# thu-nics/MixDQ

Hardware: AMD Instinct MI355X
Metric: sdxl_turbo_unet_w8a8_images_per_sec (higher is better)
Workload: dtype int8; 1 GPU; sdxl_turbo_unet_w8a8_1024px_bs1_1step; global_batch=1, per_gpu_batch=1, px=1024, latent=128, unet_forwards_per_image=1, unet_rows_per_image=1, graphs_cached=1, w_config=weight/uniform_8, a_config=act/act_8.00, bos=True, parallelism=dp1 (batch-sharded replicas, no step-loop collective), hip_graph=True, producer_fusions=True, swap_glue=False, w4_kernel_layers=0, quantizable_layers=794

## Files before the change

mixdq_amd/csrc/iconv.hip:

```cpp
#include <type_traits>

#include "iconv.h"

namespace mixdq {
namespace {

__device__ uint4 g_zero_page;

__device__ __forceinline__ void dma16(const void* gsrc, char* lds_wave_base) {
  __builtin_amdgcn_global_load_lds((const __attribute__((address_space(1))) void*)gsrc,
                                   (__attribute__((address_space(3))) void*)lds_wave_base, 16, 0, 0);
}

__device__ __forceinline__ uint32_t add_f16x2_(uint32_t a, uint32_t b) {
  const v2h ah = *reinterpret_cast<const v2h*>(&a), bh = *reinterpret_cast<const v2h*>(&b);
  v2f r = __builtin_convertvector(ah, v2f) + __builtin_convertvector(bh, v2f);
  asm("" : "+v"(r));
  const v2h h = __builtin_convertvector(r, v2h);
  return *reinterpret_cast<const uint32_t*>(&h);
}

template <int TH, int TW, int BN, int CK, int WNG = 1, bool W4 = false>
struct HaloGeom {
  static constexpr int BM = TH * TW;
  static constexpr int HWP = TW + 2, HP = (TH + 2) * HWP;
  static constexpr int KSPLIT = CK / 64;
  static constexpr int NWAVES = 8, NTHREADS = 512, WPX = NWAVES / KSPLIT / WNG;
  static constexpr int PPP = 1024 / CK, LPP = CK / 16;
  static constexpr int H_NI = ((HP + PPP - 1) / PPP + NWAVES - 1) / NWAVES;
  static constexpr int HALO_BYTES = H_NI * NWAVES * 1024;
  static constexpr int WROW = W4 ? CK / 2 : CK, WLPP = WROW / 16;
  static constexpr int W_TAP = BN * WROW;
  static constexpr int W_PIECES = (3 * W_TAP + 1023) / 1024;
  static constexpr int W_STAGE = W_PIECES * 1024;
  static constexpr int W_LO = W_PIECES / NWAVES, W_REM = W_PIECES % NWAVES, W_NI = W_LO + (W_REM ? 1 : 0);
  static constexpr int HALO_OFF = 3 * W_STAGE;
  static constexpr int MAIN_BYTES = HALO_OFF + 2 * HALO_BYTES;
  static constexpr int CS_STRIDE = BN * 2 + 16;
  static constexpr int WTN = BN / WNG;
  static constexpr int WTM = BM / WPX, TM = WTM / 16, TN = WTN / 16;
  static constexpr int PART_BYTES = (KSPLIT - 1) * WPX * TM * TN * 4 * 64 * 4;
  static constexpr int SMEM = MAIN_BYTES + 9 * BN * 4 + BN * 6;
  static_assert(CK == 64 || CK == 128, "one or two 64-byte MFMA k-steps per chunk");
  static_assert((W4 || W_TAP % 1024 == 0) && W_TAP % 256 == 0 && WTN % 16 == 0 && WTM % 16 == 0,
                "whole DMA pieces (int8) / LDS bank rows / MFMA tiles");
  static_assert(WNG == 1 || KSPLIT == 1, "channel wave groups only without the k-split");
  static_assert(BM * CS_STRIDE + PART_BYTES <= MAIN_BYTES, "epilogue staging overlays the main buffers");
  static_assert(SMEM <= 160 * 1024, "LDS is 160 KiB per CU");
  static_assert(H_NI + 2 * W_NI <= 63, "vmcnt is a 6-bit counter");
  __device__ static int swz(int row) {
    if (CK == 64) return ((row >> 2) & 1) << 1;
    return TW == 16 ? ((row >> 1) & 3) << 1 : (row >> 1) & 7;
  }
  __device__ static int wswz(int row) { return WROW == 64 ? (row >> 2) & 3 : (row >> 3) & 1; }
};

template <int TH, int TW, int BN, int CK, int WNG = 1, bool W4 = false>
__global__ __launch_bounds__(512, 2) void conv3x3_halo_kernel(const HaloConvArgs p) {
  using G = HaloGeom<TH, TW, BN, CK, WNG, W4>;
  constexpr int BM = G::BM, HWP = G::HWP, HP = G::HP, TM = G::TM, TN = G::TN;
  constexpr int CS_STRIDE = G::CS_STRIDE;
  MIXDQ_ARGS_NOW(p.X, p.Wt, p.scale, p.bias, p.table, p.zp, p.D, p.res, p.res_div, p.NI, p.H, p.W, p.C,
                 p.K, p.unfused, p.ups);
  const float zpv = *(const __attribute__((address_space(4))) float*)p.zp;
  extern __shared__ __attribute__((aligned(16))) char smem[];
  const int tid = threadIdx.x, lane = tid & 63;
  const int wid = __builtin_amdgcn_readfirstlane(tid >> 6);
  const int kg = WNG == 1 ? wid / G::WPX : 0;
  const int wn = WNG == 1 ? 0 : wid / G::WPX;
  const int wm = wid % G::WPX;
  const int lrow = lane & 15, lkq = lane >> 4;

  const int tiles_x = p.W / TW, tiles_y = p.H / TH, tiles_n = (p.K + BN - 1) / BN;
  const int tiles_m = p.NI * tiles_y * tiles_x;
  const int nwg = tiles_m * tiles_n;
  const int bid = blockIdx.x;
  const int xcd = bid % kNumXCD, q8 = nwg / kNumXCD, r8 = nwg % kNumXCD;
  const int wg = (xcd < r8 ? xcd * (q8 + 1) : r8 * (q8 + 1) + (xcd - r8) * q8) + bid / kNumXCD;
  constexpr int GM = 8;
  const int per_group = GM * tiles_n;
  const int group = wg / per_group;
  const int first_m = group * GM;
  const int gsz = min(GM, tiles_m - first_m);
  const int rem = wg - group * per_group;
  const int tile_n = rem / gsz, tile_m = first_m + (rem - tile_n * gsz);
  const int img = tile_m / (tiles_y * tiles_x);
  const int trem = tile_m - img * (tiles_y * tiles_x);
  const int y0 = (trem / tiles_x) * TH, x0 = (trem % tiles_x) * TW;
  const int n0 = tile_n * BN;
  const int C = p.C;
  const int nch = (C + CK - 1) / CK;
  const char* zero = reinterpret_cast<const char*>(&g_zero_page);
  const int sh = p.ups ? 1 : 0, SW = p.W >> sh;
  const int8_t* ximg = p.X + (int64_t)img * (p.H >> sh) * SW * C;

  const bool has_bias = p.bias != nullptr;
  v4f pre_tab, pre_sc;
  uint2 pre_bs;
  const bool tab_on = tid < 9 * (BN / 4), pre_on = tid < BN / 4;
  const int tab_q = tid % (BN / 4), tab_c = tid / (BN / 4);
  const bool tab_in = n0 + tab_q * 4 < p.K;
  if (tab_on) {
    const int rc = tab_c / 3, cc = tab_c % 3;
    const int rlo = rc == 1 ? 1 : 0, rhi = rc == 2 ? 1 : 2, slo = cc == 1 ? 1 : 0, shi = cc == 2 ? 1 : 2;
    const int cls = ((rlo * 3 + rhi) * 3 + slo) * 3 + shi;
    const int n = tab_in ? n0 + tab_q * 4 : 0;
    pre_tab = *reinterpret_cast<const v4f*>(p.table + (int64_t)cls * p.K + n);
    if (pre_on) {
      pre_sc = *reinterpret_cast<const v4f*>(p.scale + n);
      if (has_bias) pre_bs = *reinterpret_cast<const uint2*>(p.bias + n);
    }
  }

  uint32_t h_off[G::H_NI];
  int h_c16[G::H_NI];
  bool h_ok[G::H_NI];
#pragma unroll
  for (int j = 0; j < G::H_NI; ++j) {
    const int h = (wid + 8 * j) * G::PPP + lane / G::LPP;
    const int hy = h / HWP, hx = h - hy * HWP;
    const int iy = y0 - 1 + hy, ix = x0 - 1 + hx;
    const int c16 = ((lane % G::LPP) ^ G::swz(h)) << 4;
    h_ok[j] = h < HP && (unsigned)iy < (unsigned)p.H && (unsigned)ix < (unsigned)p.W;
    h_off[j] = h_ok[j] ? (uint32_t)((iy >> sh) * SW + (ix >> sh)) * (uint32_t)C + c16 : 0u;
    h_c16[j] = c16;
  }
  uint32_t w_off[G::W_NI];
  int w_c16[G::W_NI];
  bool w_ok[G::W_NI];
#pragma unroll
  for (int j = 0; j < G::W_NI; ++j) {
    const int q = wid + 8 * j;
    if constexpr (W4) {
      const int L = q * 64 + lane;
      const int s = L / (BN * G::WLPP), rem = L - s * (BN * G::WLPP);
      const int row = rem / G::WLPP;
      const int c16 = ((rem % G::WLPP) ^ G::wswz(row)) << 4;
      w_ok[j] = L < 3 * BN * G::WLPP && n0 + row < p.K;
      w_off[j] = w_ok[j] ? (uint32_t)(n0 + row) * (uint32_t)(9 * (C >> 1)) + (uint32_t)(s * (C >> 1)) + c16 : 0u;
      w_c16[j] = c16;
    } else {
      const int s = q / (BN / G::PPP), row = (q - s * (BN / G::PPP)) * G::PPP + lane / G::LPP;
      const int c16 = ((lane % G::LPP) ^ G::swz(row)) << 4;
      w_ok[j] = q < G::W_PIECES && n0 + row < p.K;
      w_off[j] = w_ok[j] ? (uint32_t)(n0 + row) * (uint32_t)(9 * C) + (uint32_t)(s * C) + c16 : 0u;
      w_c16[j] = c16;
    }
  }
  auto stage_halo = [&](int chunk, int buf) {
    char* dst = smem + G::HALO_OFF + buf * G::HALO_BYTES;
    const int c0 = chunk * CK;
    const bool live = chunk < nch;
#pragma unroll
    for (int j = 0; j < G::H_NI; ++j) {
      const bool ok = live && h_ok[j] && c0 + h_c16[j] < C;
      dma16(ok ? (const void*)(ximg + h_off[j] + c0) : (const void*)zero, dst + (wid + 8 * j) * 1024);
    }
  };
  auto stage_w = [&](int chunk, int r) {
    char* dst = smem + r * G::W_STAGE;
    const int c0 = W4 ? chunk * (CK / 2) : chunk * CK;
    const int cend = W4 ? C >> 1 : C;
    const bool live = chunk < nch;
    const int8_t* base = p.Wt + (r * 3) * cend + c0;
#pragma unroll
    for (int j = 0; j < G::W_NI; ++j) {
      if (j >= G::W_LO && wid >= G::W_REM) continue;
      const bool ok = live && w_ok[j] && c0 + w_c16[j] < cend;
      dma16(ok ? (const void*)(base + w_off[j]) : (const void*)zero, dst + (wid + 8 * j) * 1024);
    }
  };
  auto wait_row = [&](auto r_c) {
    constexpr int r = decltype(r_c)::value;
    constexpr int extra = r == 1 ? G::H_NI : 0;
    if constexpr (G::W_REM == 0) {
      asm volatile("s_waitcnt vmcnt(%0)\n\ts_barrier" ::"n"(G::W_LO + extra) : "memory");
    } else {
      if (wid < G::W_REM) asm volatile("s_waitcnt vmcnt(%0)\n\ts_barrier" ::"n"(G::W_NI + extra) : "memory");
      else asm volatile("s_waitcnt vmcnt(%0)\n\ts_barrier" ::"n"(G::W_LO + extra) : "memory");
    }
  };

  int x_rd[TM][9];
#pragma unroll
  for (int t = 0; t < TM; ++t) {
    const int i = wm * G::WTM + t * 16 + lrow;
    const int hb = (i / TW) * HWP + (i % TW);
#pragma unroll
    for (int tap = 0; tap < 9; ++tap) {
      const int h = hb + (tap / 3) * HWP + (tap % 3);
      x_rd[t][tap] = G::HALO_OFF + h * CK + (((kg * 4 + lkq) ^ G::swz(h)) << 4);
    }
  }
  int w_rd[TN];
#pragma unroll
  for (int tn = 0; tn < TN; ++tn) {
    const int row = wn * G::WTN + tn * 16 + lrow;
    if constexpr (W4)
      w_rd[tn] = row * G::WROW + (((kg * 2 + (lkq >> 1)) ^ G::wswz(row)) << 4) + (lkq & 1) * 8;
    else
      w_rd[tn] = row * CK + (((kg * 4 + lkq) ^ G::swz(row)) << 4);
  }
  v4i acc[TN][TM];
#pragma unroll
  for (int a = 0; a < TN; ++a)
#pragma unroll
    for (int b = 0; b < TM; ++b) acc[a][b] = v4i{0, 0, 0, 0};

  stage_halo(0, 0);
  stage_w(0, 0);
  stage_w(0, 1);
  auto chunk_body = [&](auto hb_c, int ch) {
    constexpr int HB = decltype(hb_c)::value;
#pragma unroll
    for (int r = 0; r < 3; ++r) {
      if (r == 0) wait_row(std::integral_constant<int, 0>{});
      else if (r == 1) wait_row(std::integral_constant<int, 1>{});
      else wait_row(std::integral_constant<int, 2>{});
      if (r == 0) stage_halo(ch + 1, HB ^ 1);
      stage_w(ch + (r + 2) / 3, (r + 2) % 3);
      const char* Ws = smem + r * G::W_STAGE;
      const char* Hs = smem + HB * G::HALO_BYTES;
#pragma unroll
      for (int s = 0; s < 3; ++s) {
        v4i wf[TN], xf[TM];
#pragma unroll
        for (int t = 0; t < TM; ++t) xf[t] = *reinterpret_cast<const v4i*>(Hs + x_rd[t][r * 3 + s]);
#pragma unroll
        for (int tn = 0; tn < TN; ++tn) {
          if constexpr (W4) {
            const uint2 w = *reinterpret_cast<const uint2*>(Ws + s * G::W_TAP + w_rd[tn]);
            wf[tn] = v4i{(int)(w.x & 0xF0F0F0F0u), (int)((w.x << 4) & 0xF0F0F0F0u),
                         (int)(w.y & 0xF0F0F0F0u), (int)((w.y << 4) & 0xF0F0F0F0u)};
          } else {
            wf[tn] = *reinterpret_cast<const v4i*>(Ws + s * G::W_TAP + w_rd[tn]);
          }
        }
#pragma unroll
        for (int tn = 0; tn < TN; ++tn)
#pragma unroll
          for (int t = 0; t < TM; ++t)
            acc[tn][t] = __builtin_amdgcn_mfma_i32_16x16x64_i8(wf[tn], xf[t], acc[tn][t], 0, 0, 0);
      }
    }
  };
  for (int ch = 0; ch < nch; ch += 2) {
    chunk_body(std::integral_constant<int, 0>{}, ch);
    if (ch + 1 < nch) chunk_body(std::integral_constant<int, 1>{}, ch + 1);
  }
  asm volatile("s_waitcnt vmcnt(0)" ::: "memory");

  constexpr int PARAM_OFF = G::MAIN_BYTES;
  float* P_TAB = reinterpret_cast<float*>(smem + PARAM_OFF);
  float* P_SC = P_TAB + 9 * BN;
  __half* P_BS = reinterpret_cast<__half*>(P_SC + BN);
  if (tab_on) {
    const v4f zero4 = {0.f, 0.f, 0.f, 0.f};
    if constexpr (W4) {
      pre_tab = pre_tab * 16.0f;
      if (pre_on) pre_sc = pre_sc * 0.0625f;
    }
    *reinterpret_cast<v4f*>(P_TAB + tab_c * BN + tab_q * 4) = tab_in ? pre_tab : zero4;
    if (pre_on) {
      *reinterpret_cast<v4f*>(P_SC + tab_q * 4) = tab_in ? pre_sc : zero4;
      *reinterpret_cast<uint2*>(P_BS + tab_q * 4) = tab_in && has_bias ? pre_bs : make_uint2(0u, 0u);
    }
  }
  __syncthreads();
  if constexpr (G::KSPLIT == 2) {
    constexpr int WREGS = TN * TM * 4;
    int* part = reinterpret_cast<int*>(smem + BM * CS_STRIDE) + (wm * WREGS * 64 + lane);
    if (kg != 0) {
#pragma unroll
      for (int a = 0; a < TN; ++a)
#pragma unroll
        for (int b = 0; b < TM; ++b)
#pragma unroll
          for (int e = 0; e < 4; ++e) part[((a * TM + b) * 4 + e) * 64] = acc[a][b][e];
    }
    __syncthreads();
    if (kg == 0) {
#pragma unroll
      for (int a = 0; a < TN; ++a)
#pragma unroll
        for (int b = 0; b < TM; ++b)
#pragma unroll
          for (int e = 0; e < 4; ++e) acc[a][b][e] += part[((a * TM + b) * 4 + e) * 64];
    }
  }
  char* Cs = smem;
  auto to_tile = [&](auto mode_c) {
    constexpr int MODE = decltype(mode_c)::value;
#pragma unroll
    for (int t = 0; t < TM; ++t) {
      const int ml = wm * G::WTM + t * 16 + lrow;
      const int pp = y0 + ml / TW, qq = x0 + ml % TW;
      const int rc = pp == 0 ? 1 : (pp == p.H - 1 ? 2 : 0), cc = qq == 0 ? 1 : (qq == p.W - 1 ? 2 : 0);
      const float* b0row = P_TAB + (rc * 3 + cc) * BN;
#pragma unroll
      for (int tn = 0; tn < TN; ++tn) {
        const int nl = wn * G::WTN + tn * 16 + 4 * lkq;
        v4f b0 = *reinterpret_cast<const v4f*>(b0row + nl);
        b0 = b0 * zpv;
        const v4f sc = *reinterpret_cast<const v4f*>(P_SC + nl);
        v4f bs = {0.f, 0.f, 0.f, 0.f};
        if constexpr (MODE != 0)
          bs = __builtin_convertvector(*reinterpret_cast<const v4h*>(P_BS + nl), v4f);
        uint32_t packed[2];
#pragma unroll
        for (int e2 = 0; e2 < 2; ++e2) {
          v2f x = {(float)acc[tn][t][2 * e2], (float)acc[tn][t][2 * e2 + 1]};
          const v2f b0e = {b0[2 * e2], b0[2 * e2 + 1]};
          const v2f sce = {sc[2 * e2], sc[2 * e2 + 1]};
          const v2f bse = {bs[2 * e2], bs[2 * e2 + 1]};
          v2f r;
          x = x - b0e;
          if constexpr (MODE == 0) r = x * sce;
          else if constexpr (MODE == 2) r = x * sce + bse;
          else r = __builtin_elementwise_fma(x, sce, bse);
          asm("" : "+v"(r));
          const v2h h = __builtin_convertvector(r, v2h);
          packed[e2] = *reinterpret_cast<const uint32_t*>(&h);
        }
        *reinterpret_cast<uint2*>(Cs + ml * CS_STRIDE + nl * 2) = make_uint2(packed[0], packed[1]);
      }
    }
  };
  if (kg == 0) {
    if (!has_bias) to_tile(std::integral_constant<int, 0>{});
    else if (!p.unfused) to_tile(std::integral_constant<int, 1>{});
    else to_tile(std::integral_constant<int, 2>{});
  }
  constexpr int CPRO = BN / 8;
  const bool n8 = (p.K & 7) == 0;
  constexpr int ST_ITERS = (BM * CPRO + G::NTHREADS - 1) / G::NTHREADS;
  static_assert(ST_ITERS <= 10, "residual chunks parked in registers");
  v4i res_late[ST_ITERS];
  const bool res_late_on = p.res != nullptr && n8;
  if (res_late_on) {
#pragma unroll
    for (int it = 0; it < ST_ITERS; ++it) {
      const int idx = min(tid + it * G::NTHREADS, BM * CPRO - 1);
      const int row = idx / CPRO, cc = idx - row * CPRO;
      const int n = n0 + cc * 8 < p.K ? n0 + cc * 8 : 0;
      const int64_t pix = ((int64_t)img * p.H + (y0 + row / TW)) * p.W + (x0 + row % TW);
      res_late[it] = *reinterpret_cast<const v4i*>(p.res + (p.res_div == 1 ? pix : (int64_t)img) * p.K + n);
    }
  }
  __syncthreads();
#pragma unroll
  for (int it = 0; it < ST_ITERS; ++it) {
    const int idx = tid + it * G::NTHREADS;
    if (idx >= BM * CPRO) break;
    const int row = idx / CPRO, cc = idx - row * CPRO;
    const int n = n0 + cc * 8;
    if (n >= p.K) continue;
    const int64_t pix = ((int64_t)img * p.H + (y0 + row / TW)) * p.W + (x0 + row % TW);
    uint4 v = *reinterpret_cast<const uint4*>(Cs + row * CS_STRIDE + cc * 16);
    if (p.res != nullptr) {
      const __half* rp = p.res + (p.res_div == 1 ? pix : (int64_t)img) * p.K + n;
      uint32_t rw[4];
      if (n8) {
        const v4i r = res_late[it];
        rw[0] = (uint32_t)r[0]; rw[1] = (uint32_t)r[1]; rw[2] = (uint32_t)r[2]; rw[3] = (uint32_t)r[3];
      } else {
        const uint2 r0 = *reinterpret_cast<const uint2*>(rp);
        rw[0] = r0.x; rw[1] = r0.y; rw[2] = 0; rw[3] = 0;
        if (n + 8 <= p.K) {
          const uint2 r1 = *reinterpret_cast<const uint2*>(rp + 4);
          rw[2] = r1.x; rw[3] = r1.y;
        }
      }
      uint32_t* vw = reinterpret_cast<uint32_t*>(&v);
#pragma unroll
      for (int e = 0; e < 4; ++e) vw[e] = add_f16x2_(vw[e], rw[e]);
    }
    __half* dst = p.D + pix * p.K + n;
    if (n8) {
      const v4i vv = {(int)v.x, (int)v.y, (int)v.z, (int)v.w};
        __builtin_nontemporal_store(vv, reinterpret_cast<v4i*>(dst));
    } else {
      *reinterpret_cast<uint2*>(dst) = make_uint2(v.x, v.y);
      if (n + 8 <= p.K) *reinterpret_cast<uint2*>(dst + 4) = make_uint2(v.z, v.w);
    }
  }
}

template <int TH, int TW, int BN, int CK, int WNG = 1, bool W4 = false>
int launch_halo(const HaloConvArgs& a, hipStream_t stream) {
  using G = HaloGeom<TH, TW, BN, CK, WNG, W4>;
  static bool seen[64] = {};
  if (const int st = lds_opt_in(reinterpret_cast<const void*>(&conv3x3_halo_kernel<TH, TW, BN, CK, WNG, W4>),
                                G::SMEM, seen))
    return st;
  const int64_t grid = (int64_t)a.NI * (a.H / TH) * (a.W / TW) * ((a.K + BN - 1) / BN);
  if (grid <= 0 || grid > 0x7fffffff) return MIXDQ_ERR_INVALID_ARG;
  conv3x3_halo_kernel<TH, TW, BN, CK, WNG, W4><<<dim3((unsigned)grid), 512, G::SMEM, stream>>>(a);
  return launch_status();
}

}

int halo_conv_select(int NI, int H, int W, int C, int K, int R, int S, int stride, int pad, bool w4) {
  if (R != 3 || S != 3 || stride != 1 || pad != 1 || NI <= 0) return 0;
  if (C % 64 != 0 || K % 4 != 0 || H % 8 != 0 || W % 8 != 0) return 0;
  if ((int64_t)H * W * C >= (1ll << 32) || (int64_t)K * 9 * C >= (1ll << 32)) return 0;
  const int64_t tiles_n = (K + 79) / 80;
  if (H % 16 == 0 && W % 16 == 0 && K % 160 == 0 && (int64_t)NI * (H / 16) * (W / 16) * (K / 160) >= kNumCU)
    return 93;
  if (H % 16 == 0 && W % 16 == 0 && (int64_t)NI * (H / 16) * (W / 16) * tiles_n >= kNumCU) return 92;
  if (w4 && K <= 16) return 0;
  if (W % 16 == 0 && (int64_t)NI * (H / 8) * (W / 16) * tiles_n >= kNumCU) return 90;
  return 91;
}

int halo_conv_launch(const HaloConvArgs& a, int tile, hipStream_t stream, bool w4) {
  if (w4) {
    switch (tile) {
#define X(ID, TH, TW, BN, CK, WNG) case ID: return launch_halo<TH, TW, BN, CK, WNG, true>(a, stream);
      MIXDQ_HALO_TILES(X)
#undef X
      default: return MIXDQ_ERR_INVALID_ARG;
    }
  }
  switch (tile) {
#define X(ID, TH, TW, BN, CK, WNG) case ID: return launch_halo<TH, TW, BN, CK, WNG>(a, stream);
    MIXDQ_HALO_TILES(X)
#undef X
    default: return MIXDQ_ERR_INVALID_ARG;
  }
}

}
```

Before: 92.23 images/s.

## Software-pipeline LDS fragment reads across taps in halo int8 conv kernel

Adds a pipelined main loop for the 3x3 halo convolution that double-buffers MFMA fragments in registers. It issues LDS reads for the next tap (via inline ds_read with immediate offsets) while MFMAs for the current tap run, and uses explicit lgkmcnt waits. Tile 92 also gets a fourth weight stage, and tile 90 staggers DMA issue across wave halves. The first global-to-LDS requests are hoisted ahead of the epilogue parameter loads, and compile-time timestamp probes are added but off by default. The aim is to hide LDS latency and DMA issue behind MFMA work, at the cost of more registers, more LDS for the extra stage, and tighter counter budgets.

```diff
diff --git a/mixdq_amd/csrc/iconv.hip b/mixdq_amd/csrc/iconv.hip
--- a/mixdq_amd/csrc/iconv.hip
+++ b/mixdq_amd/csrc/iconv.hip
@@ -1,11 +1,57 @@
 #include <type_traits>
+#include <utility>
 
 #include "iconv.h"
+
+#ifndef MIXDQ_STAMP
+#define MIXDQ_STAMP 0
+#endif
+#ifndef MIXDQ_HALO_PIPE
+#define MIXDQ_HALO_PIPE -1
+#endif
 
 namespace mixdq {
 namespace {
 
 __device__ uint4 g_zero_page;
+#if MIXDQ_STAMP
+__device__ unsigned long long g_halo_stamps;
+#define MIXDQ_HALO_STAMP(slot)                                                                    \
+  do {                                                                                            \
+    const unsigned long long t_ = __builtin_amdgcn_s_memtime();                                   \
+    const unsigned long long r_ = __builtin_amdgcn_s_memrealtime();                               \
+    const unsigned long long a_ = g_halo_stamps;                                                  \
+    if (a_ != 0 && (threadIdx.x & 63) == 0) {                                                     \
+      auto sp_ = (__attribute__((address_space(1))) unsigned long long*)a_ +                      \
+                 ((size_t)blockIdx.x * 16 + (threadIdx.x >> 6)) * 16;                             \
+      sp_[slot] = t_;                                                                             \
+      if ((slot) == 0) sp_[8] = r_;                                                               \
+      if ((slot) == 7) sp_[9] = r_;                                                               \
+    }                                                                                             \
+  } while (0)
+#else
+#define MIXDQ_HALO_STAMP(slot) do {} while (0)
+#endif
+
+template <class F, int... I>
+__device__ __forceinline__ void static_for_(F&& f, std::integer_sequence<int, I...>) {
+  (f(std::integral_constant<int, I>{}), ...);
+}
+template <int N, class F>
+__device__ __forceinline__ void static_for(F&& f) {
+  static_for_(f, std::make_integer_sequence<int, N>{});
+}
+
+template <int OFF>
+__device__ __forceinline__ void lds_rd128(v4i& d, unsigned addr) {
+  static_assert(OFF >= 0 && OFF < 65536, "ds offset field");
+  asm volatile("ds_read_b128 %0, %1 offset:%2" : "=v"(d) : "v"(addr), "n"(OFF) : "memory");
+}
+template <int OFF>
+__device__ __forceinline__ void lds_rd64(v2i& d, unsigned addr) {
+  static_assert(OFF >= 0 && OFF < 65536, "ds offset field");
+  asm volatile("ds_read_b64 %0, %1 offset:%2" : "=v"(d) : "v"(addr), "n"(OFF) : "memory");
+}
 
 __device__ __forceinline__ void dma16(const void* gsrc, char* lds_wave_base) {
   __builtin_amdgcn_global_load_lds((const __attribute__((address_space(1))) void*)gsrc,
@@ -20,7 +66,7 @@
   return *reinterpret_cast<const uint32_t*>(&h);
 }
 
-template <int TH, int TW, int BN, int CK, int WNG = 1, bool W4 = false>
+template <int TH, int TW, int BN, int CK, int WNG = 1, bool W4 = false, int PIPE = 0>
 struct HaloGeom {
   static constexpr int BM = TH * TW;
   static constexpr int HWP = TW + 2, HP = (TH + 2) * HWP;
@@ -34,7 +80,8 @@
   static constexpr int W_PIECES = (3 * W_TAP + 1023) / 1024;
   static constexpr int W_STAGE = W_PIECES * 1024;
   static constexpr int W_LO = W_PIECES / NWAVES, W_REM = W_PIECES % NWAVES, W_NI = W_LO + (W_REM ? 1 : 0);
-  static constexpr int HALO_OFF = 3 * W_STAGE;
+  static constexpr int WST = PIPE == 2 ? 4 : 3;
+  static constexpr int HALO_OFF = WST * W_STAGE;
   static constexpr int MAIN_BYTES = HALO_OFF + 2 * HALO_BYTES;
   static constexpr int CS_STRIDE = BN * 2 + 16;
   static constexpr int WTN = BN / WNG;
@@ -47,7 +94,8 @@
   static_assert(WNG == 1 || KSPLIT == 1, "channel wave groups only without the k-split");
   static_assert(BM * CS_STRIDE + PART_BYTES <= MAIN_BYTES, "epilogue staging overlays the main buffers");
   static_assert(SMEM <= 160 * 1024, "LDS is 160 KiB per CU");
-  static_assert(H_NI + 2 * W_NI <= 63, "vmcnt is a 6-bit counter");
+  static_assert(H_NI + (WST - 1) * W_NI <= 63, "vmcnt is a 6-bit counter");
+  static_assert(PIPE == 0 || 2 * (TM + TN) <= 15, "lgkmcnt is a 4-bit counter: two taps of fragment reads in flight");
   __device__ static int swz(int row) {
     if (CK == 64) return ((row >> 2) & 1) << 1;
     return TW == 16 ? ((row >> 1) & 3) << 1 : (row >> 1) & 7;
@@ -55,13 +103,14 @@
   __device__ static int wswz(int row) { return WROW == 64 ? (row >> 2) & 3 : (row >> 3) & 1; }
 };
 
-template <int TH, int TW, int BN, int CK, int WNG = 1, bool W4 = false>
+template <int TH, int TW, int BN, int CK, int WNG = 1, bool W4 = false, int PIPE = 0, bool STAG = false>
 __global__ __launch_bounds__(512, 2) void conv3x3_halo_kernel(const HaloConvArgs p) {
-  using G = HaloGeom<TH, TW, BN, CK, WNG, W4>;
-  constexpr int BM = G::BM, HWP = G::HWP, HP = G::HP, TM = G::TM, TN = G::TN;
+  using G = HaloGeom<TH, TW, BN, CK, WNG, W4, PIPE>;
+  constexpr int BM = G::BM, HWP = G::HWP, HP = G::HP, TM = G::TM, TN = G::TN, WST = G::WST;
   constexpr int CS_STRIDE = G::CS_STRIDE;
   MIXDQ_ARGS_NOW(p.X, p.Wt, p.scale, p.bias, p.table, p.zp, p.D, p.res, p.res_div, p.NI, p.H, p.W, p.C,
                  p.K, p.unfused, p.ups);
+  MIXDQ_HALO_STAMP(0);
   const float zpv = *(const __attribute__((address_space(4))) float*)p.zp;
   extern __shared__ __attribute__((aligned(16))) char smem[];
   const int tid = threadIdx.x, lane = tid & 63;
@@ -94,24 +143,6 @@
   const int sh = p.ups ? 1 : 0, SW = p.W >> sh;
   const int8_t* ximg = p.X + (int64_t)img * (p.H >> sh) * SW * C;
 
-  const bool has_bias = p.bias != nullptr;
-  v4f pre_tab, pre_sc;
-  uint2 pre_bs;
-  const bool tab_on = tid < 9 * (BN / 4), pre_on = tid < BN / 4;
-  const int tab_q = tid % (BN / 4), tab_c = tid / (BN / 4);
-  const bool tab_in = n0 + tab_q * 4 < p.K;
-  if (tab_on) {
-    const int rc = tab_c / 3, cc = tab_c % 3;
-    const int rlo = rc == 1 ? 1 : 0, rhi = rc == 2 ? 1 : 2, slo = cc == 1 ? 1 : 0, shi = cc == 2 ? 1 : 2;
-    const int cls = ((rlo * 3 + rhi) * 3 + slo) * 3 + shi;
-    const int n = tab_in ? n0 + tab_q * 4 : 0;
-    pre_tab = *reinterpret_cast<const v4f*>(p.table + (int64_t)cls * p.K + n);
-    if (pre_on) {
-      pre_sc = *reinterpret_cast<const v4f*>(p.scale + n);
-      if (has_bias) pre_bs = *reinterpret_cast<const uint2*>(p.bias + n);
-    }
-  }
-
   uint32_t h_off[G::H_NI];
   int h_c16[G::H_NI];
   bool h_ok[G::H_NI];
@@ -157,8 +188,8 @@
       dma16(ok ? (const void*)(ximg + h_off[j] + c0) : (const void*)zero, dst + (wid + 8 * j) * 1024);
     }
   };
-  auto stage_w = [&](int chunk, int r) {
-    char* dst = smem + r * G::W_STAGE;
+  auto stage_w = [&](int chunk, int r, int stage) {
+    char* dst = smem + stage * G::W_STAGE;
     const int c0 = W4 ? chunk * (CK / 2) : chunk * CK;
     const int cend = W4 ? C >> 1 : C;
     const bool live = chunk < nch;
@@ -181,6 +212,33 @@
     }
   };
 
+  auto first_requests = [&]() {
+    stage_halo(0, 0);
+#pragma unroll
+    for (int r = 0; r < WST - 1; ++r) stage_w(0, r, r);
+    __builtin_amdgcn_sched_barrier(0);
+    MIXDQ_HALO_STAMP(1);
+  };
+  if constexpr (PIPE != 0) first_requests();
+
+  const bool has_bias = p.bias != nullptr;
+  v4f pre_tab, pre_sc;
+  uint2 pre_bs;
+  const bool tab_on = tid < 9 * (BN / 4), pre_on = tid < BN / 4;
+  const int tab_q = tid % (BN / 4), tab_c = tid / (BN / 4);
+  const bool tab_in = n0 + tab_q * 4 < p.K;
+  if (tab_on) {
+    const int rc = tab_c / 3, cc = tab_c % 3;
+    const int rlo = rc == 1 ? 1 : 0, rhi = rc == 2 ? 1 : 2, slo = cc == 1 ? 1 : 0, shi = cc == 2 ? 1 : 2;
+    const int cls = ((rlo * 3 + rhi) * 3 + slo) * 3 + shi;
+    const int n = tab_in ? n0 + tab_q * 4 : 0;
+    pre_tab = *reinterpret_cast<const v4f*>(p.table + (int64_t)cls * p.K + n);
+    if (pre_on) {
+      pre_sc = *reinterpret_cast<const v4f*>(p.scale + n);
+      if (has_bias) pre_bs = *reinterpret_cast<const uint2*>(p.bias + n);
+    }
+  }
+
   int x_rd[TM][9];
 #pragma unroll
   for (int t = 0; t < TM; ++t) {
@@ -206,19 +264,108 @@
   for (int a = 0; a < TN; ++a)
 #pragma unroll
     for (int b = 0; b < TM; ++b) acc[a][b] = v4i{0, 0, 0, 0};
-
-  stage_halo(0, 0);
-  stage_w(0, 0);
-  stage_w(0, 1);
+  if constexpr (PIPE == 0) first_requests();
+
+  [[maybe_unused]] v4i xf2[2][TM];
+  [[maybe_unused]] std::conditional_t<W4, v2i, v4i> wf2[2][TN];
+  const unsigned lds0 = (unsigned)(size_t)(__attribute__((address_space(3))) char*)smem;
+  auto rd_x = [&](auto hb_c, auto tap_c, auto buf_c) {
+    static_for<TM>([&](auto t) {
+      lds_rd128<decltype(hb_c)::value * G::HALO_BYTES>(xf2[decltype(buf_c)::value][decltype(t)::value],
+                                                        lds0 + x_rd[decltype(t)::value][decltype(tap_c)::value]);
+    });
+  };
+  auto rd_w = [&](auto s_c, auto buf_c, unsigned stage_base) {
+    static_for<TN>([&](auto tn) {
+      const unsigned a = lds0 + stage_base + w_rd[decltype(tn)::value];
+      if constexpr (W4) lds_rd64<decltype(s_c)::value * G::W_TAP>(wf2[decltype(buf_c)::value][decltype(tn)::value], a);
+      else lds_rd128<decltype(s_c)::value * G::W_TAP>(wf2[decltype(buf_c)::value][decltype(tn)::value], a);
+    });
+  };
+  auto land = [&](auto n_c, auto buf_c) {
+    asm volatile("s_waitcnt lgkmcnt(%0)" ::"n"(decltype(n_c)::value) : "memory");
+    constexpr int B = decltype(buf_c)::value;
+#pragma unroll
+    for (int t = 0; t < TM; ++t) asm volatile("" : "+v"(xf2[B][t]));
+#pragma unroll
+    for (int tn = 0; tn < TN; ++tn) asm volatile("" : "+v"(wf2[B][tn]));
+    __builtin_amdgcn_sched_barrier(0);
+  };
+  auto mma = [&](auto buf_c) {
+    constexpr int B = decltype(buf_c)::value;
+#pragma unroll
+    for (int tn = 0; tn < TN; ++tn) {
+      v4i w;
+      if constexpr (W4) {
+        const uint32_t lo = (uint32_t)wf2[B][tn][0], hi = (uint32_t)wf2[B][tn][1];
+        w = v4i{(int)(lo & 0xF0F0F0F0u), (int)((lo << 4) & 0xF0F0F0F0u),
+                (int)(hi & 0xF0F0F0F0u), (int)((hi << 4) & 0xF0F0F0F0u)};
+      } else {
+        w = wf2[B][tn];
+      }
+#pragma unroll
+      for (int t = 0; t < TM; ++t)
+        acc[tn][t] = __builtin_amdgcn_mfma_i32_16x16x64_i8(w, xf2[B][t], acc[tn][t], 0, 0, 0);
+    }
+    __builtin_amdgcn_sched_barrier(0);
+  };
+  auto pipe_step = [&](auto hb_c, auto r_c, int ch) {
+    constexpr int HB = decltype(hb_c)::value, R = decltype(r_c)::value;
+    constexpr int P0 = (HB + R) & 1;
+    using B0 = std::integral_constant<int, P0>;
+    using B1 = std::integral_constant<int, P0 ^ 1>;
+    using HBc = std::integral_constant<int, HB>;
+    constexpr int NF = TM + TN;
+    const int g = 3 * ch + R;
+    auto requests = [&]() {
+      if (R == 0) stage_halo(ch + 1, HB ^ 1);
+      if constexpr (WST == 3) stage_w(ch + (R + 2) / 3, (R + 2) % 3, (R + 2) % 3);
+      else stage_w(ch + 1, R, (g + 3) & 3);
+    };
+    const bool late = STAG && wid >= 4;
+    if (!late) requests();
+    const unsigned wbase = (WST == 3 ? R : (g & 3)) * G::W_STAGE;
+    if constexpr (PIPE != 2) rd_w(std::integral_constant<int, 0>{}, B0{}, wbase);
+    rd_x(HBc{}, std::integral_constant<int, R * 3 + 1>{}, B1{});
+    rd_w(std::integral_constant<int, 1>{}, B1{}, wbase);
+    land(std::integral_constant<int, NF>{}, B0{});
+    mma(B0{});
+    if (late) requests();
+    rd_x(HBc{}, std::integral_constant<int, R * 3 + 2>{}, B0{});
+    rd_w(std::integral_constant<int, 2>{}, B0{}, wbase);
+    land(std::integral_constant<int, NF>{}, B1{});
+    mma(B1{});
+    constexpr int NP = PIPE == 2 ? NF : TM;
+    const unsigned wnext = ((g + 1) & 3) * G::W_STAGE;
+    if constexpr (R < 2) rd_x(HBc{}, std::integral_constant<int, (R + 1) * 3>{}, B1{});
+    else rd_x(std::integral_constant<int, HB ^ 1>{}, std::integral_constant<int, 0>{}, B1{});
+    if constexpr (PIPE == 2) rd_w(std::integral_constant<int, 0>{}, B1{}, wnext);
+    land(std::integral_constant<int, NP>{}, B0{});
+    mma(B0{});
+    wait_row(std::integral_constant<int, (R + 1) % 3>{});
+  };
+  auto pipe_first = [&]() {
+    wait_row(std::integral_constant<int, 0>{});
+    MIXDQ_HALO_STAMP(2);
+    rd_x(std::integral_constant<int, 0>{}, std::integral_constant<int, 0>{}, std::integral_constant<int, 0>{});
+    if constexpr (PIPE == 2) rd_w(std::integral_constant<int, 0>{}, std::integral_constant<int, 0>{}, 0u);
+  };
   auto chunk_body = [&](auto hb_c, int ch) {
     constexpr int HB = decltype(hb_c)::value;
+    if constexpr (PIPE != 0) {
+      pipe_step(hb_c, std::integral_constant<int, 0>{}, ch);
+      pipe_step(hb_c, std::integral_constant<int, 1>{}, ch);
+      pipe_step(hb_c, std::integral_constant<int, 2>{}, ch);
+      return;
+    }
 #pragma unroll
     for (int r = 0; r < 3; ++r) {
       if (r == 0) wait_row(std::integral_constant<int, 0>{});
       else if (r == 1) wait_row(std::integral_constant<int, 1>{});
       else wait_row(std::integral_constant<int, 2>{});
+      if (r == 0 && HB == 0 && ch == 0) MIXDQ_HALO_STAMP(2);
       if (r == 0) stage_halo(ch + 1, HB ^ 1);
-      stage_w(ch + (r + 2) / 3, (r + 2) % 3);
+      stage_w(ch + (r + 2) / 3, (r + 2) % 3, (r + 2) % 3);
       const char* Ws = smem + r * G::W_STAGE;
       const char* Hs = smem + HB * G::HALO_BYTES;
 #pragma unroll
@@ -244,11 +391,17 @@
       }
     }
   };
+  if constexpr (PIPE != 0) pipe_first();
   for (int ch = 0; ch < nch; ch += 2) {
     chunk_body(std::integral_constant<int, 0>{}, ch);
     if (ch + 1 < nch) chunk_body(std::integral_constant<int, 1>{}, ch + 1);
   }
   asm volatile("s_waitcnt vmcnt(0)" ::: "memory");
+  if constexpr (PIPE != 0) {
+    land(std::integral_constant<int, 0>{}, std::integral_constant<int, 0>{});
+    land(std::integral_constant<int, 0>{}, std::integral_constant<int, 1>{});
+  }
+  MIXDQ_HALO_STAMP(3);
 
   constexpr int PARAM_OFF = G::MAIN_BYTES;
   float* P_TAB = reinterpret_cast<float*>(smem + PARAM_OFF);
@@ -331,6 +484,7 @@
     else if (!p.unfused) to_tile(std::integral_constant<int, 1>{});
     else to_tile(std::integral_constant<int, 2>{});
   }
+  MIXDQ_HALO_STAMP(5);
   constexpr int CPRO = BN / 8;
   const bool n8 = (p.K & 7) == 0;
   constexpr int ST_ITERS = (BM * CPRO + G::NTHREADS - 1) / G::NTHREADS;
@@ -384,22 +538,56 @@
       if (n + 8 <= p.K) *reinterpret_cast<uint2*>(dst + 4) = make_uint2(v.z, v.w);
     }
   }
-}
-
-template <int TH, int TW, int BN, int CK, int WNG = 1, bool W4 = false>
-int launch_halo(const HaloConvArgs& a, hipStream_t stream) {
-  using G = HaloGeom<TH, TW, BN, CK, WNG, W4>;
+  MIXDQ_HALO_STAMP(7);
+}
+
+constexpr int halo_pipe(int id, bool w4) {
+  if (id == 93) return 0;
+  const bool room4 = !w4 && (id == 92 || id == 91);
+  if (MIXDQ_HALO_PIPE >= 0) return MIXDQ_HALO_PIPE == 2 && !room4 ? 1 : MIXDQ_HALO_PIPE;
+  return !w4 && id == 92 ? 2 : 1;
+}
+
+#ifndef MIXDQ_HALO_STAGGER
+#define MIXDQ_HALO_STAGGER -1
+#endif
+constexpr bool halo_stagger(int id, bool w4) {
+  if (halo_pipe(id, w4) == 0) return false;
+  if (MIXDQ_HALO_STAGGER >= 0) return MIXDQ_HALO_STAGGER != 0;
+  return id == 90;
+}
+
+template <int TH, int TW, int BN, int CK, int WNG, bool W4, int PIPE, bool STAG>
+int launch_halo_form(const HaloConvArgs& a, int64_t grid, hipStream_t stream) {
+  using G = HaloGeom<TH, TW, BN, CK, WNG, W4, PIPE>;
   static bool seen[64] = {};
-  if (const int st = lds_opt_in(reinterpret_cast<const void*>(&conv3x3_halo_kernel<TH, TW, BN, CK, WNG, W4>),
+  if (const int st = lds_opt_in(reinterpret_cast<const void*>(&conv3x3_halo_kernel<TH, TW, BN, CK, WNG, W4, PIPE, STAG>),
                                 G::SMEM, seen))
     return st;
+  conv3x3_halo_kernel<TH, TW, BN, CK, WNG, W4, PIPE, STAG><<<dim3((unsigned)grid), 512, G::SMEM, stream>>>(a);
+  return launch_status();
+}
+
+template <int ID, int TH, int TW, int BN, int CK, int WNG = 1, bool W4 = false>
+int launch_halo(const HaloConvArgs& a, hipStream_t stream) {
+  constexpr int PIPE = halo_pipe(ID, W4);
+  constexpr bool STAG = halo_stagger(ID, W4);
   const int64_t grid = (int64_t)a.NI * (a.H / TH) * (a.W / TW) * ((a.K + BN - 1) / BN);
   if (grid <= 0 || grid > 0x7fffffff) return MIXDQ_ERR_INVALID_ARG;
-  conv3x3_halo_kernel<TH, TW, BN, CK, WNG, W4><<<dim3((unsigned)grid), 512, G::SMEM, stream>>>(a);
-  return launch_status();
-}
-
-}
+  if constexpr (W4 && ID == 92 && PIPE != 0 && MIXDQ_HALO_PIPE < 0) {
+    if (grid > kNumCU) return launch_halo_form<TH, TW, BN, CK, WNG, W4, 0, false>(a, grid, stream);
+  }
+  return launch_halo_form<TH, TW, BN, CK, WNG, W4, PIPE, STAG>(a, grid, stream);
+}
+
+}
+
+#if MIXDQ_STAMP
+extern "C" int mixdq_debug_stamps_halo(void* buffer) {
+  const unsigned long long b = (unsigned long long)(uintptr_t)buffer;
+  return hipMemcpyToSymbol(HIP_SYMBOL(g_halo_stamps), &b, sizeof(b)) == hipSuccess ? MIXDQ_OK : MIXDQ_ERR_LAUNCH;
+}
+#endif
 
 int halo_conv_select(int NI, int H, int W, int C, int K, int R, int S, int stride, int pad, bool w4) {
   if (R != 3 || S != 3 || stride != 1 || pad != 1 || NI <= 0) return 0;
@@ -417,14 +605,14 @@
 int halo_conv_launch(const HaloConvArgs& a, int tile, hipStream_t stream, bool w4) {
   if (w4) {
     switch (tile) {
-#define X(ID, TH, TW, BN, CK, WNG) case ID: return launch_halo<TH, TW, BN, CK, WNG, true>(a, stream);
+#define X(ID, TH, TW, BN, CK, WNG) case ID: return launch_halo<ID, TH, TW, BN, CK, WNG, true>(a, stream);
       MIXDQ_HALO_TILES(X)
 #undef X
       default: return MIXDQ_ERR_INVALID_ARG;
     }
   }
   switch (tile) {
-#define X(ID, TH, TW, BN, CK, WNG) case ID: return launch_halo<TH, TW, BN, CK, WNG>(a, stream);
+#define X(ID, TH, TW, BN, CK, WNG) case ID: return launch_halo<ID, TH, TW, BN, CK, WNG>(a, stream);
     MIXDQ_HALO_TILES(X)
 #undef X
     default: return MIXDQ_ERR_INVALID_ARG;
```

Measured after the change: 92.53 images/s, median of 6. About the same (+0.3%).
